# IndigoPurple/DEQSCI

Hardware: AMD Instinct MI355X
Metric: reconstructed frames/sec at 256x256x8, 180 DEQ iters (higher is better)
Workload: dtype f32 (tensors and accumulation; the 64->64 layers' products as split-fp16 MFMAs, see arithmetic)

## Files before the change

deqsci_amd/_hip.py:

```python
import ctypes
import math
import os

import torch

LAYOUT_HWB = 0
LAYOUT_BHW = 1
MAX_M = 8
PART_STRIDE = MAX_M + 1
BN_TRAIN_CHUNK, BN_TRAIN_MAX_WG = 128, 1024
WGRAD_CHAIN = 4096

_LIB_PATH = os.environ.get("DEQSCI_HIP_LIB") or os.path.join(os.path.dirname(os.path.abspath(__file__)), "lib", "libdeqsci_hip.so")
_lib = None

_i64, _int, _f32, _ptr = ctypes.c_int64, ctypes.c_int, ctypes.c_float, ctypes.c_void_p
_f64 = ctypes.c_double

SIGNATURES = {
    "deqsci_sci_forward_f32": [_ptr, _ptr, _ptr, _i64, _i64, _i64, _i64, _int, _int, _ptr],
    "deqsci_sci_adjoint_f32": [_ptr, _ptr, _ptr, _i64, _i64, _i64, _i64, _int, _int, _ptr],
    "deqsci_phi_sum_f32": [_ptr, _ptr, _i64, _i64, _i64, _i64, _int, _ptr],
    "deqsci_gap_update_f32": [_ptr, _ptr, _ptr, _ptr, _ptr, _i64, _i64, _i64, _i64, _int, _int, _int, _ptr],
    "deqsci_gap_update_grad_f32": [_ptr, _ptr, _ptr, _ptr, _ptr, _ptr, _ptr, _ptr, _ptr, _i64, _i64, _i64, _i64, _int, _int, _ptr],
# ... 8 lines not shown
    "deqsci_residual_store_ref_f32": [_ptr, _ptr, _ptr, _ptr, _ptr, _ptr, _ptr, _ptr, _i64, _i64, _int, _int, _int, _ptr],
    "deqsci_anderson_apply_solve_ref_f32": [_ptr, _ptr, _ptr, _ptr, _ptr, _ptr, _i64, _i64, _int, _int, _int, _int, _f32, _f32, _ptr],
    "deqsci_gram_ref_fusable": [_i64, _i64],
    "deqsci_gram_row_chain16_f32": [_ptr, _ptr, _ptr, _i64, _i64, _int, _int, _int, _int, _ptr],
    "deqsci_anderson_mix_f32": [_ptr, _ptr, _ptr, _ptr, _f32, _int, _i64, _i64, _int, _ptr],
    "deqsci_anderson_mix_gap_f32": [_ptr, _ptr, _ptr, _f32, _int, _int, _ptr, _ptr, _ptr, _ptr, _ptr,
                                    _i64, _i64, _i64, _i64, _int, _int, _ptr],
    "deqsci_anderson_mix_gap_timed_f32": [_ptr, _ptr, _ptr, _f32, _int, _int, _ptr, _ptr, _ptr, _ptr, _ptr,
                                          _i64, _i64, _i64, _i64, _int, _int, _ptr, _ptr, _ptr],
    "deqsci_bias_relu_f32": [_ptr, _ptr, _i64, _i64, _i64, _int, _int, _ptr],
    "deqsci_ffdnet_tail_f32": [_ptr, _ptr, _ptr, _ptr, _i64, _i64, _i64, _ptr],
    "deqsci_ffdnet_head_f32": [_ptr, _ptr, _ptr, _i64, _ptr, _i64, _i64, _i64, _ptr],
    "deqsci_conv3x3_c64_to_1_f32": [_ptr, _ptr, _ptr, _ptr, _i64, _i64, _i64, _ptr],
    "deqsci_conv3x3_c1_to_64_f32": [_ptr, _ptr, _ptr, _i64, _i64, _i64, _int, _ptr],
    "deqsci_conv3x3_c64_winograd_f32": [_ptr, _ptr, _ptr, _ptr, _i64, _i64, _i64, _int, _ptr],
    "deqsci_conv3x3_c64_winograd_timed_f32": [_ptr, _ptr, _ptr, _ptr, _i64, _i64, _i64, _int, _ptr, _ptr, _ptr],
    "deqsci_conv3x3_c64_winograd44_f32": [_ptr, _ptr, _ptr, _ptr, _i64, _i64, _i64, _int, _ptr],
    "deqsci_conv3x3_c64_winograd44_timed_f32": [_ptr, _ptr, _ptr, _ptr, _i64, _i64, _i64, _int, _ptr, _ptr, _ptr],
    "deqsci_conv3x3_c64_winograd44_layout_f32": [_ptr, _ptr, _ptr, _ptr, _i64, _i64, _i64, _int, _int, _int, _ptr, _ptr, _ptr],
    "deqsci_conv3x3_c64_split16": [_ptr, _ptr, _ptr, _ptr, _i64, _i64, _i64, _int, _int, _ptr, _int, _ptr, _int, _ptr, _int, _ptr, _ptr, _ptr],
    "deqsci_conv3x3_c64_split16_stack": [_ptr, _ptr, _ptr, _ptr, _int, _i64, _i64, _i64, _ptr, _i64, _int, _int, _ptr, _ptr, _ptr, _ptr],
    "deqsci_conv3x3_c64_wino16": [_ptr, _ptr, _ptr, _ptr, _i64, _i64, _i64, _int, _int, _ptr, _int, _ptr, _int, _ptr, _ptr, _ptr],
    "deqsci_conv3x3_c64_wino16_stack": [_ptr, _ptr, _ptr, _ptr, _int, _i64, _i64, _i64, _ptr, _i64, _int, _int, _ptr, _ptr, _ptr, _ptr],
    "deqsci_f32_to_split16": [_ptr, _ptr, _i64, _i64, _i64, _ptr, _int, _ptr],
    "deqsci_absmax_f32": [_ptr, _i64, _i64, _ptr, _ptr],
    "deqsci_ffdnet_tail_split16": [_ptr, _ptr, _ptr, _i64, _i64, _i64, _int, _ptr, _int, _ptr],
    "deqsci_ffdnet_head_split16": [_ptr, _ptr, _ptr, _i64, _ptr, _i64, _i64, _i64, _int, _ptr, _int, _ptr, _int, _ptr, _ptr],
    "deqsci_conv3x3_c64_to_1_split16": [_ptr, _ptr, _ptr, _i64, _i64, _i64, _int, _ptr, _int, _ptr],
    "deqsci_conv3x3_c64_to_1_p32": [_ptr, _ptr, _ptr, _i64, _i64, _i64, _int, _ptr, _int, _ptr],
    "deqsci_conv3x3_c1_to_64_p32": [_ptr, _ptr, _ptr, _i64, _i64, _i64, _int, _ptr, _int, _ptr, _ptr],
    "deqsci_ffdnet_head_p32": [_ptr, _ptr, _ptr, _i64, _ptr, _i64, _i64, _i64, _int, _ptr, _int, _ptr, _int, _ptr],
    "deqsci_ffdnet_tail_p32": [_ptr, _ptr, _ptr, _i64, _i64, _i64, _int, _ptr, _int, _ptr],
    "deqsci_conv3x3_c1_to_64_sp16": [_ptr, _ptr, _ptr, _i64, _i64, _i64, _int, _ptr, _int, _ptr, _ptr],
    "deqsci_ssim_f32": [_ptr, _ptr, _ptr, _i64, _i64, _i64, _i64, _int, _int, _int, _int, _ptr, _ptr],
    "deqsci_sqerr_rows_f32": [_ptr, _ptr, _ptr, _i64, _i64, _i64, _int, _ptr, _ptr],
    "deqsci_gaptv_f32": [_ptr, _ptr, _ptr, _ptr, _i64, _i64, _i64, _i64, _int, _int, _f64, _f64, _f64, _int, _ptr, _ptr, _ptr],
    "deqsci_tv_chambolle_f32": [_ptr, _ptr, _i64, _i64, _i64, _f64, _f64, _int, _f64, _ptr, _ptr, _ptr],
    "deqsci_relu_mask_pack_f32": [_ptr, _ptr, _i64, _ptr],
    "deqsci_conv3x3_c64_winograd_masked_f32": [_ptr, _ptr, _ptr, _ptr, _i64, _i64, _i64, _ptr],
    "deqsci_conv3x3_c1_to_64_masked_f32": [_ptr, _ptr, _ptr, _ptr, _i64, _i64, _i64, _ptr],
    "deqsci_ffdnet_head_masked_f32": [_ptr, _ptr, _ptr, _ptr, _i64, _i64, _i64, _ptr],
    "deqsci_power_step_f32": [_ptr, _ptr, _ptr, _ptr, _i64, _i64, _ptr, _ptr],
    "deqsci_broyden_dots_f32": [_ptr, _ptr, _ptr, _ptr, _ptr, _ptr, _ptr, _i64, _i64, _int, _int, _ptr],
    "deqsci_broyden_update_f32": [_ptr, _ptr, _ptr, _ptr, _ptr, _ptr, _ptr, _ptr, _ptr, _ptr, _i64, _i64, _int, _int, _int, _ptr],
    "deqsci_epsilon2_norms_f32": [_ptr, _ptr, _ptr, _ptr, _ptr, _i64, _i64, _ptr],
    "deqsci_epsilon2_update_f32": [_ptr, _ptr, _ptr, _ptr, _ptr, _ptr, _i64, _i64, _f32, _ptr],
    "deqsci_wgrad3x3_c64_c64_f32": [_ptr, _ptr, _ptr, _i64, _i64, _i64, _ptr, _ptr],
    "deqsci_wgrad3x3_c1_c64_f32": [_ptr, _ptr, _ptr, _int, _i64, _i64, _i64, _ptr, _ptr],
    "deqsci_wgrad3x3_c64_c64_bn_f32": [_ptr, _ptr, _ptr, _ptr, _ptr, _ptr, _ptr, _i64, _i64, _i64, _ptr, _ptr],
    "deqsci_wgrad3x3_shuffle_f32": [_ptr, _ptr, _i64, _ptr, _ptr, _int, _i64, _i64, _i64, _ptr, _ptr],
    "deqsci_realsn_power_f32": [_ptr, _ptr, _ptr, _ptr, _ptr, _int, _f32, _f32, _i64, _i64, _i64, _i64, _ptr, _ptr],
    "deqsci_realsn_grad_f32": [_ptr, _ptr, _ptr, _ptr, _ptr, _ptr, _f32, _i64, _i64, _i64, _i64, _ptr, _ptr],
    "deqsci_bn_train_stats_f32": [_ptr, _ptr, _ptr, _ptr, _ptr, _f64, _i64, _ptr, _ptr],
    "deqsci_bn_train_apply_f32": [_ptr, _ptr, _ptr, _ptr, _f64, _ptr, _ptr, _int, _i64, _ptr],
    "deqsci_bn_train_grad_stats_f32": [_ptr, _ptr, _ptr, _f64, _ptr, _ptr, _ptr, _i64, _ptr, _ptr],
    "deqsci_bn_train_grad_apply_f32": [_ptr, _ptr, _ptr, _ptr, _ptr, _f64, _ptr, _i64, _ptr],
    "deqsci_event_create": [ctypes.POINTER(_ptr)],
    "deqsci_event_destroy": [_ptr],
    "deqsci_event_elapsed_ms": [_ptr, _ptr, ctypes.POINTER(_f32)],
}
OTHER_EXPORTS = ("deqsci_version", "deqsci_error_string", "deqsci_anderson_chunks",
                 "deqsci_partials_bytes", "deqsci_gram_bytes", "deqsci_gram_ref_bytes", "deqsci_ssim_workspace_bytes",
                 "deqsci_gaptv_workspace_bytes", "deqsci_tv_chambolle_workspace_bytes", "deqsci_sqerr_workspace_bytes", "deqsci_power_workspace_bytes",
                 "deqsci_broyden_workspace_bytes", "deqsci_broyden_chunk", "deqsci_epsilon2_workspace_bytes", "deqsci_epsilon2_chunk",
                 "deqsci_wgrad_workspace_bytes", "deqsci_wgrad_bn_workspace_bytes", "deqsci_realsn_workspace_bytes",
                 "deqsci_bn_train_workspace_bytes")


class DeqsciHipError(RuntimeError):
    pass


def lib_path():
    return _LIB_PATH


def load():
    global _lib
    if _lib is not None:
        return _lib
    if not os.path.exists(_LIB_PATH):
        raise DeqsciHipError(
            f"{_LIB_PATH} is missing: build it with `make` (or __graft_entry__.build()). "
            "deqsci_amd has no CPU / eager fallback for its HIP kernels.")
    lib = ctypes.CDLL(_LIB_PATH, mode=ctypes.RTLD_GLOBAL)
    for name, argtypes in SIGNATURES.items():
        fn = getattr(lib, name)
        fn.argtypes = argtypes
        fn.restype = _int
# ... 14 lines not shown
    lib.deqsci_sqerr_workspace_bytes.argtypes = [_i64, _i64]
    lib.deqsci_power_workspace_bytes.restype = ctypes.c_size_t
    lib.deqsci_power_workspace_bytes.argtypes = [_i64, _i64]
    lib.deqsci_broyden_workspace_bytes.restype = ctypes.c_size_t
    lib.deqsci_broyden_workspace_bytes.argtypes = [_i64, _i64, _int]
    lib.deqsci_broyden_chunk.restype = _i64
    lib.deqsci_broyden_chunk.argtypes = []
    lib.deqsci_epsilon2_workspace_bytes.restype = ctypes.c_size_t
    lib.deqsci_epsilon2_workspace_bytes.argtypes = [_i64, _i64]
    lib.deqsci_epsilon2_chunk.restype = _i64
    lib.deqsci_epsilon2_chunk.argtypes = []
    lib.deqsci_wgrad_workspace_bytes.restype = ctypes.c_size_t
    lib.deqsci_wgrad_workspace_bytes.argtypes = [_i64, _i64, _i64]
    lib.deqsci_wgrad_bn_workspace_bytes.restype = ctypes.c_size_t
    lib.deqsci_wgrad_bn_workspace_bytes.argtypes = [_i64, _i64, _i64]
    lib.deqsci_realsn_workspace_bytes.restype = ctypes.c_size_t
    lib.deqsci_realsn_workspace_bytes.argtypes = [_i64, _i64, _i64, _i64]
    lib.deqsci_bn_train_workspace_bytes.restype = ctypes.c_size_t
    lib.deqsci_bn_train_workspace_bytes.argtypes = [_i64]
    lib.deqsci_gaptv_workspace_bytes.restype = _i64
    lib.deqsci_gaptv_workspace_bytes.argtypes = [_i64, _i64, _i64, _i64]
    lib.deqsci_tv_chambolle_workspace_bytes.restype = _i64
    lib.deqsci_tv_chambolle_workspace_bytes.argtypes = [_i64, _i64, _i64]
    _lib = lib
    return lib


def _check(code, what):
    if code != 0:
        msg = load().deqsci_error_string(code).decode()
        raise DeqsciHipError(f"{what} failed with code {code}: {msg}")


def _p(t, name="tensor", allow_none=False):
    if t is None:
        if allow_none:
            return None
        raise DeqsciHipError(f"{name} is None")
    if not isinstance(t, torch.Tensor) or not t.is_cuda:
        raise DeqsciHipError(f"{name} must be a torch tensor on a HIP device (got "
                             f"{getattr(t, 'device', type(t))}); deqsci_amd has no CPU path")
    if t.dtype != torch.float32:
        raise DeqsciHipError(f"{name} must be float32, got {t.dtype}")
    if not t.is_contiguous():
        raise DeqsciHipError(f"{name} must be contiguous")
    return t.data_ptr()
# ... 925 lines not shown
            raise DeqsciHipError("conv3x3_c64_split16: a measuring launch (track=) serves the sp16 output")
        with _dev(x.t):
            _check(load().deqsci_conv3x3_c64_split16(x.t.data_ptr(), wp.data_ptr(), _p(bias, "bias", True), None, n, H, W, 1 if relu else 0,
                                                     weights.sw, _rng(x.rng, n), x.exp, None, 0, _rng(track, n), 0, _stream(), None, None),
                   "conv3x3_c64_split16 (measuring)")
        return None
    if out_f32:
        o = out if out is not None else torch.empty((n, 64, H, W), dtype=torch.float32, device=dev, memory_format=torch.channels_last)
        ot = o
    else:
        o = out if out is not None else Sp16.empty(n, H, W, dev)
        o.rng, o.exp = out_rng, int(out_exp)
        ot = o.t
    ev = _hook_events("s16", n, H, W, events) or (None, None)
    with _dev(x.t):
        _check(load().deqsci_conv3x3_c64_split16(x.t.data_ptr(), wp.data_ptr(), _p(bias, "bias", True), ot.data_ptr(), n, H, W, 1 if relu else 0,
                                                 weights.sw, _rng(x.rng, n), x.exp, _rng(out_rng, n), int(out_exp), None, 1 if out_f32 else 0,
                                                 _stream(), ev[0], ev[1]), "conv3x3_c64_split16")
    return o


class _Stack:
    __slots__ = ("table", "n_layers", "keep", "_state")

    def __init__(self, layers, device):
        rows, keep = [], []
        for w16, bias, relu in layers:
            if not isinstance(w16, self.WEIGHTS):
                raise DeqsciHipError(f"{type(self).__name__}: every layer needs {self.WEIGHTS.__name__}")
            wp = w16.packed if w16.packed.device == torch.device(device) else w16.packed.to(device)
            b = None if bias is None else f32c(bias.detach().to(device))
            if b is not None and b.numel() < 64:
                raise DeqsciHipError(f"{type(self).__name__}: bias must have 64 elements")
            keep += [wp, b]
            rows += [wp.data_ptr(), 0 if b is None else b.data_ptr(), (int(w16.sw) & 0xffffffff) | ((1 if relu else 0) << 32)]
        self.table = torch.tensor(rows, dtype=torch.int64).to(device)
        self.n_layers, self.keep, self._state = len(layers), keep, {}

    def state(self, n, H, W):
        st = self._state.get(("out", n, H, W))
        if st is None:
            dev = self.table.device
            for key in [k for k in self._state if k[0] == "out"]:
                del self._state[key]
            st = self._state[("out", n, H, W)] = (self.ACT.empty(n, H, W, dev), self.ACT.empty(n, H, W, dev))
        return st

    def head_buffer(self, n, H, W):
        hb = self._state.get(("head", n, H, W))
        if hb is None:
            for key in [k for k in self._state if k[0] == "head"]:
                del self._state[key]
            hb = self._state[("head", n, H, W)] = self.ACT.empty(n, H, W, self.table.device)
        return hb

    def flags(self, n, H, W):
        fl = self._state.get(("flags", n, H, W))
        if fl is None:
            n_tiles = n * (-(-H // self.TILE[0])) * (-(-W // self.TILE[1]))
            fl = self._state[("flags", n, H, W)] = torch.zeros(32 * (n_tiles + 1), dtype=torch.int32, device=self.table.device)
        return fl

    def timed_out(self):
        bad = False
        for key, fl in self._state.items():
            if key[0] == "flags" and int(fl[-32]) != 0:
                fl.zero_()
                bad = True
        return bad


STACK_SLICE_BYTES = 128 << 20


def split16_stack_per_launch(n, H, W, slice_bytes=STACK_SLICE_BYTES, cus=None, tile=(16, 32)):
    per = max(1, int(slice_bytes) // (H * W * 256))
    if cus:
        tiles = (-(-H // tile[0])) * (-(-W // tile[1]))
        unit = int(cus) // math.gcd(tiles, int(cus))
        if per >= unit:
            per -= per % unit
    return min(per, n)


def conv3x3_c64_split16_stack(x, stack, ranges=None, events=None, per_launch=None, rng_offset=0, out_bufs=None, check=None):
    if not isinstance(x, Sp16) or not isinstance(stack, Split16Stack) or not x.t.is_contiguous() or x.t.dtype != torch.float16 or not x.t.is_cuda:
        raise DeqsciHipError("conv3x3_c64_split16_stack: a contiguous Sp16 GPU activation and a Split16Stack are required")
    return _stack_launch("conv3x3_c64_split16_stack", x, stack, ranges, events, per_launch, rng_offset, out_bufs, check)


# ... 549 lines not shown
```

deqsci_amd/csrc/conv_w16.hip:

```cpp
#include "common.hpp"
#include <hip/hip_ext.h>
#include <type_traits>
#pragma clang diagnostic ignored "-Winline-asm"

namespace deqsci {
namespace w16 {

typedef _Float16 h8 __attribute__((ext_vector_type(8)));
typedef float f32x16 __attribute__((ext_vector_type(16)));
typedef float f32x4 __attribute__((ext_vector_type(4)));
typedef float f32x2 __attribute__((ext_vector_type(2)));
typedef int i32x4 __attribute__((ext_vector_type(4)));
typedef unsigned u32x4 __attribute__((ext_vector_type(4)));
typedef __attribute__((address_space(3))) char lds_char;
typedef __attribute__((address_space(3))) u32x4 lds_u32x4;
typedef __attribute__((address_space(3))) f32x4 lds_f32x4;

constexpr int WAVES = 8, TBW = 64 * WAVES;
constexpr int OUT_ROWS = 8, OUT_COLS = 64, RAW_ROWS = 10, RAW_COLS = 66, RAW_HALF = 33, RAW_PIX = RAW_ROWS * RAW_COLS;
constexpr int PLANE_B = RAW_PIX * 16;
constexpr int RAW_SLOTS = 4 * RAW_PIX;
constexpr int RAW_TOTAL = 42;
constexpr int RAW_INSTR = 6;
constexpr int RAW_BUF = RAW_TOTAL * 1024;
constexpr int W_FRAGS = 2 * 3 * 2 * 2;
constexpr int W_HALF = W_FRAGS * 1024;
constexpr int W_INSTR = W_FRAGS / WAVES;
constexpr uint32_t RAW_OOB = 0x80000000u;

__device__ __forceinline__ float sub1(float a, float b) { float r; asm("v_sub_f32 %0, %1, %2" : "=v"(r) : "v"(a), "v"(b)); return r; }
__device__ __forceinline__ float add1(float a, float b) { float r; asm("v_add_f32 %0, %1, %2" : "=v"(r) : "v"(a), "v"(b)); return r; }

__device__ __forceinline__ f32x2 pk_add(f32x2 a, f32x2 b) { f32x2 r; asm("v_pk_add_f32 %0, %1, %2" : "=v"(r) : "v"(a), "v"(b)); return r; }
__device__ __forceinline__ f32x2 pk_sub(f32x2 a, f32x2 b) { f32x2 r; asm("v_pk_add_f32 %0, %1, %2 neg_lo:[0,1] neg_hi:[0,1]" : "=v"(r) : "v"(a), "v"(b)); return r; }
__device__ __forceinline__ f32x2 pk_fma(f32x2 a, f32x2 b, f32x2 c) { f32x2 r; asm("v_pk_fma_f32 %0, %1, %2, %3" : "=v"(r) : "v"(a), "v"(b), "v"(c)); return r; }

struct StackLayer { const char* w; const float* bias; int w_exp; int relu; };
constexpr unsigned STACK_SPIN_LIMIT = 1u << 21;
constexpr int STACK_POLLS = 8;
constexpr int STACK_FLAG_STRIDE = 32;

template <int STACK>
__global__ __launch_bounds__(TBW, 2) void conv_w16_kernel(const char* __restrict__ x, const char* __restrict__ Wp, const float* __restrict__ bias,
                                                          char* __restrict__ y, int H, int W, int relu, int w_exp, const float* __restrict__ in_amax, int in_exp,
                                                          const float* __restrict__ out_amax, int out_exp, int tiles_x, int tiles_y,
                                                          int n_tiles, uint32_t mg_img, uint32_t sh_img, uint32_t mg_tx, uint32_t sh_tx,
                                                          char* __restrict__ y2, const StackLayer* __restrict__ layers, int n_layers, unsigned* flags,
                                                          int range_stride) {
    __shared__ __attribute__((aligned(16))) char Raw[2 * RAW_BUF];
    __shared__ __attribute__((aligned(16))) char Wt[2 * W_HALF];
    __shared__ __attribute__((aligned(16))) float bias_s[STACK ? 128 : 64];
    __shared__ uint32_t ready_s;
    __shared__ uint32_t poll_s[64];
    __shared__ uint32_t voff_s[RAW_INSTR * TBW];
    const int lane = (int)(threadIdx.x & 63);
    const int wave = (int)uniform((uint32_t)(threadIdx.x >> 6));
    int t_first, t_step, t_end;
    {
        const int nb = (int)gridDim.x, b = (int)blockIdx.x;
        if ((nb & 7) == 0) {
            const int per_xcd = (n_tiles + 7) >> 3;
            t_first = (b & 7) * per_xcd + (b >> 3);
            t_step = nb >> 3;
            t_end = min(n_tiles, ((b & 7) + 1) * per_xcd);
        } else { t_first = b; t_step = nb; t_end = n_tiles; }
    }
    if (t_first >= t_end) return;
    const int Wq = tiles_x * OUT_COLS;
    const int64_t HW = (int64_t)H * Wq;
    const int pl = lane & 31, kb = lane >> 5;
    const bool six = wave < RAW_TOTAL - 8 * (RAW_INSTR - 1);
    auto wait_all_but_a_tile = [&]() __attribute__((always_inline)) {
        if (six) asm volatile("s_waitcnt vmcnt(%0)" ::"n"(RAW_INSTR) : "memory");
        else asm volatile("s_waitcnt vmcnt(%0)" ::"n"(RAW_INSTR - 1) : "memory");
    };

    i32x4 rsrc;
    int ft_py0 = 0, ft_px0 = 0;
    auto fetch_tile_uniform = [&](int t, const char* xb) __attribute__((always_inline)) {
        const int n = mdiv(t, mg_img, sh_img), r = t - n * (tiles_x * tiles_y);
        const int by = mdiv(r, mg_tx, sh_tx), bx = r - by * tiles_x;
        const uint64_t base = (uint64_t)(xb + (int64_t)n * HW * 256);
        rsrc.x = (int)uniform((uint32_t)base);
        rsrc.y = (int)uniform((uint32_t)(base >> 32));
        rsrc.z = (int)uniform((uint32_t)(HW * 256));
        rsrc.w = 0x00020000;
        ft_py0 = OUT_ROWS * by - 1;
        ft_px0 = OUT_COLS * bx - 1;
// ... 73 lines not shown
        split_pair(va[2 * s], va[2 * s + 1], hi, lo);
        Vh[ns][0][2 * f + s] = hi; Vl[ns][0][2 * f + s] = lo;
        split_pair(vb[2 * s], vb[2 * s + 1], hi, lo);
        Vh[ns][1][2 * f + s] = hi; Vl[ns][1][2 * f + s] = lo;
    };
    auto xf_step = [&](int i, int rb, int rho, int hh, int ns) __attribute__((always_inline)) {
        if (i == 0) t_load(rb, rho, hh, 0);
        else if (i == 4 || i == 5) t_xf(i - 4, hh);
        else if (i == 6) { t_split(0, ns, 0); t_load(rb, rho, hh, 1); }
        else if (i == 7) t_split(1, ns, 0);
        else if (i == 8 || i == 9) t_xf(i - 8, hh);
        else if (i == 10 || i == 11) t_split(i - 10, ns, 1);
    };
    auto t_row = [&](int rb, int rho, int hh, int ns) __attribute__((always_inline)) {
#pragma unroll
        for (int i = 0; i < 12; ++i) xf_step(i, rb, rho, hh, ns);
    };

#ifdef W16_STAMP
    uint32_t st_sum[8] = {0, 0, 0, 0, 0, 0, 0, 0};
    uint64_t st_t = __builtin_readcyclecounter();
#define W16_MARK(i) do { const uint64_t now_ = __builtin_readcyclecounter(); st_sum[i] += (uint32_t)(now_ - st_t); st_t = now_; } while (0)
    uint32_t* st_out = reinterpret_cast<uint32_t*>(const_cast<float*>(STACK ? layers[0].bias : bias));
#else
#define W16_MARK(i) do { } while (0)
#endif
    int L = 0;
    auto tile_done = [&](int t) -> Done {
        Done d;
        const int n = mdiv(t, mg_img, sh_img), rr_ = t - n * (tiles_x * tiles_y);
        const int by = mdiv(rr_, mg_tx, sh_tx), bx = rr_ - by * tiles_x;
        const int ox = OUT_COLS * bx + 2 * pl;
        const uint64_t ob = (uint64_t)(y + (int64_t)n * HW * 256);
        d.orsrc.x = (int)uniform((uint32_t)ob);
        d.orsrc.y = (int)uniform((uint32_t)(ob >> 32));
        d.orsrc.z = (int)uniform((uint32_t)(HW * 256));
        d.orsrc.w = 0x00020000;
        {
            const int e_in = STACK ? (in_amax ? sp16_act_exp(in_amax[(int64_t)L * range_stride + n]) : L == 0 ? in_exp : out_exp)
                                   : in_amax ? sp16_act_exp(in_amax[n]) : in_exp;
            const int e_out = STACK ? (in_amax ? sp16_act_exp(in_amax[(int64_t)(L + 1) * range_stride + n]) : out_exp)
                                    : out_amax ? sp16_act_exp(out_amax[n]) : out_exp;
            d.oscale = sp16_pow2(e_out - e_in - w_exp);
            d.bscale = sp16_pow2(e_out);
        }
        d.oy = OUT_ROWS * by + wave;
        d.pix[0] = ox >= W ? RAW_OOB : (uint32_t)((kb * (int)HW + OUT_COLS * bx + pl) * 16);
        d.pix[1] = ox + 1 >= W ? RAW_OOB : (uint32_t)((kb * (int)HW + OUT_COLS * bx + 32 + pl) * 16);
        return d;
    };

    const char* Wnx = nullptr;
    bool s3_raw = false;
    const char* s3_w = nullptr;

    u32x4 Alo[2][2], Ahi[2][2];
    auto loadA = [&](int wbuf, int dy, int piece, int xp, int cg) __attribute__((always_inline)) {
        const u32x4 v = *reinterpret_cast<const lds_u32x4*>(abase + wbuf * W_HALF + ((((xp * 3 + dy) * 2 + piece) * 2 + cg) * 1024));
        if (piece) Alo[xp][cg] = v; else Ahi[xp][cg] = v;
    };
    auto half_stage = [&](int hs, bool wnext, bool rnext, bool raw_prev, auto&& before_barrier, auto&& shadow) __attribute__((always_inline)) {
        const int c = hs >> 1, h = hs & 1, wb = hs & 1;
        const int hn = h ^ 1, rbn = (h ? (c + 1) : c) & 1;
        auto dma = [&](int k) __attribute__((always_inline)) {
            if (k < W_INSTR) {
                if (wnext) w_piece((STACK && hs >= 6) ? s3_w : Wp, (hs + 2) & 7, wb, k);
            } else if (h == 1 && k < W_INSTR + RAW_INSTR) { if (rnext) raw_piece((c + 2) & 3, c & 1, k - W_INSTR); }
        };
        const f32x16 zero16 = {0, 0, 0, 0, 0, 0, 0, 0, 0, 0, 0, 0, 0, 0, 0, 0};
#pragma unroll
        for (int dy = 0; dy < 3; ++dy) {
            const int slot = (3 * hs + dy) & 1;
            if (dy == 2) {
                W16_MARK(h);
                if (h == 0 && raw_prev) wait_all_but_a_tile();
                else asm volatile("s_waitcnt vmcnt(0)" ::: "memory");
                W16_MARK(2 + h);
                before_barrier();
                lds_barrier();
                W16_MARK(4);
            }
#pragma unroll
            for (int i = 0; i < 12; ++i) {
                const int m = 12 * dy + i, pass = i >> 2, xp = (i >> 1) & 1, cg = i & 1, xi = 2 * h + xp;
                const bool z1st = c == 0 && dy == 0 && pass == 0;
                const h8 a = __builtin_bit_cast(h8, pass == 0 ? Alo[xp][cg] : Ahi[xp][cg]);
                const h8 b = __builtin_bit_cast(h8, pass == 1 ? Vl[slot][xp] : Vh[slot][xp]);
                acc[xi][cg] = __builtin_amdgcn_mfma_f32_32x32x16_f16(a, b, z1st ? zero16 : acc[xi][cg], 0, 0, 0);
                __builtin_amdgcn_sched_barrier(0);
// ... 53 lines not shown
    first_row_and_fragments();

    auto flag_word = [&](int t) __attribute__((always_inline)) -> const unsigned* {
        const int tpi = tiles_x * tiles_y;
        const int n = mdiv(t, mg_img, sh_img), r = t - n * tpi, by = mdiv(r, mg_tx, sh_tx), bx = r - by * tiles_x;
        const int k = lane < 9 ? lane : 4;
        const int ny = by + k / 3 - 1, nx = bx + k % 3 - 1;
        const bool ok = ny >= 0 && ny < tiles_y && nx >= 0 && nx < tiles_x;
        return flags + (int64_t)(ok ? n * tpi + ny * tiles_x + nx : t) * STACK_FLAG_STRIDE;
    };
    int pend_t = -1;
    unsigned pend_v = 0;
    f32x4 o[2][4][2];
    Done dp = {(i32x4){0, 0, 0, 0}, {RAW_OOB, RAW_OOB}, 0, 0.0f, 0.0f};
    bool have_o = false;
    auto store_step = [&](int k) __attribute__((always_inline)) {
        const int g = k >> 3, gq = (k >> 1) & 3, p = k & 1;
        if (!(dp.oy < H)) return;
        const uint32_t so = uniform((uint32_t)(2 * (4 * g + gq)) * (uint32_t)HW * 16u + (uint32_t)(dp.oy * Wq) * 16u);
        if (STACK) asm volatile("buffer_store_dwordx4 %0, %1, %2, %3 offen sc1\n\ts_nop 1" ::"v"(o[g][gq][p]), "v"(dp.pix[p]), "s"(dp.orsrc), "s"(so) : "memory");
        else asm volatile("buffer_store_dwordx4 %0, %1, %2, %3 offen nt\n\ts_nop 1" ::"v"(o[g][gq][p]), "v"(dp.pix[p]), "s"(dp.orsrc), "s"(so) : "memory");
    };
    bool raw_flying = true;
#pragma unroll 1
    for (int t_cur = t_first;;) {
        const bool new_layer = STACK && !(t_cur + t_step < t_end);
        const int t_next = new_layer ? t_first : t_cur + t_step;
        const bool next = STACK ? (!new_layer || L + 1 < n_layers) : t_next < t_end;
        const int L_next = L + (new_layer ? 1 : 0);
        const bool poll = STACK && next && L_next > 0;
        if (STACK && new_layer && next) Wnx = layers[L + 1].w;
        half_stage(0, true, false, raw_flying, nothing, [&](int m) __attribute__((always_inline)) {
            if ((m & 1) && m < 32 && have_o) store_step(m >> 1);
        });
        have_o = false;
        half_stage(1, true, true, false, nothing, [&](int m) __attribute__((always_inline)) {
            if (STACK && m == 24 && pend_t >= 0 && wave == 2 && lane == 0)
                __hip_atomic_store(flags + (int64_t)pend_t * STACK_FLAG_STRIDE, pend_v, __ATOMIC_RELAXED, __HIP_MEMORY_SCOPE_AGENT);
        });
        pend_t = -1;
        half_stage(2, true, false, true, nothing, no_shadow);
        half_stage(3, true, true, false, nothing, [&](int m) __attribute__((always_inline)) {
            if (STACK && m == 24 && wave == 0 && poll) {
                const unsigned* pf = flag_word(t_next);
                const uint32_t m0v = uniform((uint32_t)(uintptr_t)(__attribute__((address_space(3))) uint32_t*)poll_s);
                asm volatile("s_mov_b32 m0, %0\n\ts_nop 0\n\tglobal_load_lds_dword %1, off sc1" ::"s"(m0v), "v"(pf) : "m0", "memory");
            }
        });
        half_stage(4, true, false, true, [&]() __attribute__((always_inline)) {
            if (STACK && wave == 0) {
                const unsigned pv = poll_s[lane];
                const unsigned target = fbase + (unsigned)L_next;
                const bool late = poll && lane < 9 && (int)(pv - target) < 0;
                const uint32_t ok = (!poll || fgiveup) ? 1u : (__builtin_amdgcn_ballot_w64(late) == 0 ? 1u : 0u);
                if (lane == 0) ready_s = ok;
            }
        }, [&](int m) __attribute__((always_inline)) {
            if (m == 1 && next) fetch_tile_uniform(t_next, (STACK && new_layer) ? y : x);
            if (m >= 2 && m < 2 + 2 * RAW_INSTR && !(m & 1) && next) voff_set((m - 2) >> 1, fetch_lane_offset((m - 2) >> 1));
        });
        bool ready = true;
        if (STACK) {
            ready = uniform(ready_s) != 0;
            s3_raw = next && ready;
            s3_w = new_layer ? Wnx : Wp;
        }
        const bool rn = STACK ? s3_raw : next;
        half_stage(5, true, rn, false, nothing, no_shadow);
        half_stage(6, next, false, rn, nothing, no_shadow);
        half_stage(7, next, rn, false, nothing, [&](int m) __attribute__((always_inline)) { if (m == 28) dp = tile_done(t_cur); });
        raw_flying = rn;

        const bool store_now = STACK ? (!next || !ready) : !next;
        const float floor_ = relu ? 0.0f : -__builtin_inff();
        const __attribute__((address_space(3))) float* bsl = (const __attribute__((address_space(3))) float*)bias_s + (STACK ? 64 * (L & 1) : 0);
#pragma unroll
        for (int g = 0; g < 2; ++g) {
#pragma unroll
            for (int gq = 0; gq < 4; ++gq) {
                const f32x4 bz = *reinterpret_cast<const lds_f32x4*>(bsl + 32 * g + 8 * gq + 4 * kb) * dp.bscale;
#pragma unroll
                for (int k = 0; k < 4; k += 2) {
                    const int i = 4 * gq + k;
                    const f32x2 m0 = {acc[0][g][i], acc[0][g][i + 1]}, m1 = {acc[1][g][i], acc[1][g][i + 1]};
                    const f32x2 m2 = {acc[2][g][i], acc[2][g][i + 1]}, m3 = {acc[3][g][i], acc[3][g][i + 1]};
                    const f32x2 y0 = pk_add(pk_add(m0, m1), m2), y1 = pk_sub(pk_sub(m1, m2), m3);
                    const f32x2 sc = {dp.oscale, dp.oscale}, b2 = {bz[k], bz[k + 1]};
                    const f32x2 z0 = pk_fma(y0, sc, b2), z1 = pk_fma(y1, sc, b2);
                    o[g][gq][0][k] = __builtin_elementwise_maximum(z0.x, floor_);
                    o[g][gq][0][k + 1] = __builtin_elementwise_maximum(z0.y, floor_);
                    o[g][gq][1][k] = __builtin_elementwise_maximum(z1.x, floor_);
                    o[g][gq][1][k + 1] = __builtin_elementwise_maximum(z1.y, floor_);
                }
                if (store_now) { store_step(2 * (4 * g + gq)); store_step(2 * (4 * g + gq) + 1); }
            }
        }
        have_o = !store_now;
        if (rn) wait_all_but_a_tile();
        else asm volatile("s_waitcnt vmcnt(0)" ::: "memory");
        W16_MARK(5);
        if (STACK) {
            const unsigned done_v = fbase + (unsigned)(L + 1);
            if (new_layer && next) {
                const StackLayer ln = layers[L + 1];
                x = y;
                y = ((L + 1) & 1) ? y2 : y_even;
                Wp = ln.w; bias = ln.bias; w_exp = ln.w_exp; relu = ln.relu;
#ifndef W16_STAMP
                if (wave == 1) bias_s[64 * ((L + 1) & 1) + lane] = bias ? bias[lane] : 0.0f;
#endif
            }
            if (next && !ready) {
                if (have_o) {
#pragma unroll
                    for (int k = 0; k < 16; ++k) store_step(k);
                    have_o = false;
                }
                asm volatile("s_waitcnt vmcnt(0)" ::: "memory");
                __syncthreads();
                if (wave == 2 && lane == 0)
                    __hip_atomic_store(flags + (int64_t)t_cur * STACK_FLAG_STRIDE, done_v, __ATOMIC_RELAXED, __HIP_MEMORY_SCOPE_AGENT);
                if (wave == 0) {
                    const unsigned target = fbase + (unsigned)L_next;
                    const unsigned* f = flag_word(t_next);
                    if (!fgiveup) {
                        unsigned v[STACK_POLLS], spins = 0;
#pragma unroll
                        for (int q = 0; q < STACK_POLLS; ++q) {
                            asm volatile("global_load_dword %0, %1, off sc1" : "=v"(v[q]) : "v"(f) : "memory");
                            __builtin_amdgcn_s_sleep(3);
                        }
                        bool waiting = true;
// ... 5 lines not shown
                                if (++spins > STACK_SPIN_LIMIT) {
                                    fgiveup = 1;
                                    if (lane == 0) __hip_atomic_fetch_or(flags + (int64_t)n_tiles * STACK_FLAG_STRIDE, 1u, __ATOMIC_RELAXED, __HIP_MEMORY_SCOPE_AGENT);
                                    waiting = false;
                                    break;
                                }
                                asm volatile("global_load_dword %0, %1, off sc1" : "=v"(v[q]) : "v"(f) : "memory");
                                __builtin_amdgcn_s_sleep(3);
                            }
                        }
                        asm volatile("s_waitcnt vmcnt(0)" ::: "memory");
                    }
                }
                __syncthreads();
                fetch_two_chunks_and_wait();
                __syncthreads();
                first_row_and_fragments();
                raw_flying = true;
                W16_MARK(7);
            } else {
                pend_t = t_cur;
                pend_v = done_v;
            }
            if (new_layer) ++L;
        }
        if (!next) break;
        t_cur = t_next;
    }
    if (have_o) {
#pragma unroll
        for (int k = 0; k < 16; ++k) store_step(k);
    }
    asm volatile("s_waitcnt vmcnt(0)" ::: "memory");
    if (STACK) {
        __syncthreads();
        if (pend_t >= 0 && threadIdx.x == 0)
            __hip_atomic_store(flags + (int64_t)pend_t * STACK_FLAG_STRIDE, pend_v, __ATOMIC_RELAXED, __HIP_MEMORY_SCOPE_AGENT);
    }
#ifdef W16_STAMP
    W16_MARK(6);
    if (lane == 0)
        for (int i = 0; i < 8; ++i) st_out[((int)blockIdx.x * WAVES + wave) * 8 + i] = st_sum[i];
#endif
}

}
}

using namespace deqsci;

static_assert(sizeof(w16::StackLayer) == 24, "the layer table of deqsci_conv3x3_c64_wino16_stack is three 8-byte words per layer");

extern "C" int deqsci_conv3x3_c64_wino16(const void* x_p32, const void* u_packed, const float* bias, void* y_p32, int64_t n, int64_t H, int64_t W,
                                         int relu, int w_exp, const float* in_amax, int in_exp, const float* out_amax, int out_exp,
                                         deqsci_stream_t stream, void* start_event, void* stop_event) {
    if (!x_p32 || !u_packed || !y_p32) return DEQSCI_ERR_NULL;
    if ((start_event == nullptr) != (stop_event == nullptr)) return DEQSCI_ERR_NULL;
    if (n <= 0 || H <= 0 || W <= 0) return DEQSCI_ERR_SHAPE;
    if (x_p32 == y_p32 || sp16_bad_exp(w_exp) || sp16_bad_exp(in_exp) || sp16_bad_exp(out_exp)) return DEQSCI_ERR_UNSUPPORTED;
    if (!aligned16(x_p32) || !aligned16(u_packed) || !aligned16(y_p32)) return DEQSCI_ERR_ALIGN;
    const int64_t tiles_x = ceil_div(W, w16::OUT_COLS), tiles_y = ceil_div(H, w16::OUT_ROWS);
    const int64_t n_tiles = n * tiles_x * tiles_y;
    if (n_tiles > (int64_t)INT32_MAX / 16 || H * tiles_x * w16::OUT_COLS * 256 + 16 > (int64_t)w16::RAW_OOB) return DEQSCI_ERR_UNSUPPORTED;
    hipStream_t st = static_cast<hipStream_t>(stream);
    const int64_t resident = (int64_t)num_cus();
    const dim3 grid((unsigned)(n_tiles < resident ? n_tiles : resident));
    uint32_t mg_img, sh_img, mg_tx, sh_tx;
    mdiv_magic((uint32_t)(tiles_x * tiles_y), &mg_img, &sh_img);
    mdiv_magic((uint32_t)tiles_x, &mg_tx, &sh_tx);
    hipEvent_t ev0 = static_cast<hipEvent_t>(start_event), ev1 = static_cast<hipEvent_t>(stop_event);
    hipExtLaunchKernelGGL((w16::conv_w16_kernel<0>), grid, dim3(w16::TBW), 0, st, ev0, ev1, 0, static_cast<const char*>(x_p32), static_cast<const char*>(u_packed),
                          bias, static_cast<char*>(y_p32), (int)H, (int)W, relu, w_exp, in_amax, in_exp, out_amax, out_exp, (int)tiles_x,
                          (int)tiles_y, (int)n_tiles, mg_img, sh_img, mg_tx, sh_tx, static_cast<char*>(nullptr),
                          static_cast<const w16::StackLayer*>(nullptr), 1, static_cast<unsigned*>(nullptr), 0);
    return launch_status();
}

extern "C" int deqsci_conv3x3_c64_wino16_stack(const void* x_p32, void* y_even, void* y_odd, const void* layers, int n_layers,
                                               int64_t n, int64_t H, int64_t W, const float* ranges, int64_t range_stride, int in_exp, int out_exp,
                                               void* flags, deqsci_stream_t stream, void* start_event, void* stop_event) {
    if (!x_p32 || !y_even || !layers || !flags || (n_layers > 1 && !y_odd)) return DEQSCI_ERR_NULL;
    if ((start_event == nullptr) != (stop_event == nullptr)) return DEQSCI_ERR_NULL;
    if (n <= 0 || H <= 0 || W <= 0 || n_layers <= 0 || (ranges && (range_stride < n || range_stride > INT32_MAX))) return DEQSCI_ERR_SHAPE;
    if (x_p32 == y_even || x_p32 == y_odd || y_even == y_odd || n_layers > 64 || sp16_bad_exp(in_exp) || sp16_bad_exp(out_exp)) return DEQSCI_ERR_UNSUPPORTED;
    if (!aligned16(x_p32) || !aligned16(y_even) || !aligned16(y_odd) || (reinterpret_cast<uintptr_t>(layers) & 7u) || (reinterpret_cast<uintptr_t>(flags) & 3u))
        return DEQSCI_ERR_ALIGN;
    const int64_t tiles_x = ceil_div(W, w16::OUT_COLS), tiles_y = ceil_div(H, w16::OUT_ROWS);
    const int64_t n_tiles = n * tiles_x * tiles_y;
    if (H * tiles_x * w16::OUT_COLS * 256 + 16 > (int64_t)w16::RAW_OOB) return DEQSCI_ERR_UNSUPPORTED;
    if (n_tiles > (int64_t)INT32_MAX / (16 * 32)) return DEQSCI_ERR_UNSUPPORTED;
    static int occ_cache[64] = {0};
    const int64_t fit = resident_workgroups(w16::conv_w16_kernel<1>, w16::TBW, occ_cache);
    if (fit <= 0) return DEQSCI_ERR_UNSUPPORTED;
    const int64_t resident = fit < (int64_t)num_cus() ? fit : (int64_t)num_cus();
    hipStream_t st = static_cast<hipStream_t>(stream);
    uint32_t mg_img, sh_img, mg_tx, sh_tx;
    mdiv_magic((uint32_t)(tiles_x * tiles_y), &mg_img, &sh_img);
    mdiv_magic((uint32_t)tiles_x, &mg_tx, &sh_tx);
    hipEvent_t ev0 = static_cast<hipEvent_t>(start_event), ev1 = static_cast<hipEvent_t>(stop_event);
    hipExtLaunchKernelGGL((w16::conv_w16_kernel<1>), dim3((unsigned)(n_tiles < resident ? n_tiles : resident)), dim3(w16::TBW), 0, st, ev0, ev1, 0,
                          static_cast<const char*>(x_p32), static_cast<const char*>(nullptr), static_cast<const float*>(nullptr), static_cast<char*>(y_even),
                          (int)H, (int)W, 0, 0, ranges, in_exp, static_cast<const float*>(nullptr), out_exp, (int)tiles_x, (int)tiles_y, (int)n_tiles,
                          mg_img, sh_img, mg_tx, sh_tx, static_cast<char*>(y_odd), static_cast<const w16::StackLayer*>(layers), n_layers,
                          static_cast<unsigned*>(flags), (int)range_stride);
    return launch_status();
}
```

include/deqsci_hip.h:

```cpp
#ifndef DEQSCI_HIP_H
#define DEQSCI_HIP_H

#include <stddef.h>
#include <stdint.h>

#ifdef __cplusplus
extern "C" {
#endif

#define DEQSCI_LAYOUT_HWB 0
#define DEQSCI_LAYOUT_BHW 1

#define DEQSCI_MAX_M 8
#define DEQSCI_PART_STRIDE (DEQSCI_MAX_M + 1)

#define DEQSCI_ERR_NULL        (-1)
#define DEQSCI_ERR_SHAPE       (-2)
#define DEQSCI_ERR_ALIGN       (-3)
#define DEQSCI_ERR_UNSUPPORTED (-4)

typedef void* deqsci_stream_t;

const char* deqsci_version(void);
const char* deqsci_error_string(int code);
// ... 101 lines not shown

#define DEQSCI_ACT_NHWC 0
#define DEQSCI_ACT_BLK32 1
int deqsci_conv3x3_c64_winograd44_layout_f32(const float* x, const float* u_packed, const float* bias, float* y,
                                             int64_t n, int64_t H, int64_t W, int relu, int in_layout, int out_layout,
                                             deqsci_stream_t stream, void* start_event, void* stop_event);

#define DEQSCI_SP16_DEFAULT_EXP 8
#define DEQSCI_SP16_TARGET_EXP 11
int deqsci_conv3x3_c64_split16(const void* x_sp16, const void* w_packed, const float* bias, void* y,
                               int64_t n, int64_t H, int64_t W, int relu, int w_exp, const float* in_amax, int in_exp,
                               const float* out_amax, int out_exp, float* track_amax, int out_f32,
                               deqsci_stream_t stream, void* start_event, void* stop_event);
int deqsci_conv3x3_c64_split16_stack(const void* x_sp16, void* y_even, void* y_odd, const void* layers, int n_layers,
                                     int64_t n, int64_t H, int64_t W, const float* ranges, int64_t range_stride, int in_exp, int out_exp,
                                     void* flags, deqsci_stream_t stream, void* start_event, void* stop_event);
int deqsci_conv3x3_c64_wino16(const void* x_p32, const void* u_packed, const float* bias, void* y_p32,
                              int64_t n, int64_t H, int64_t W, int relu, int w_exp, const float* in_amax, int in_exp,
                              const float* out_amax, int out_exp,
                              deqsci_stream_t stream, void* start_event, void* stop_event);
int deqsci_conv3x3_c64_wino16_stack(const void* x_p32, void* y_even, void* y_odd, const void* layers, int n_layers,
                                    int64_t n, int64_t H, int64_t W, const float* ranges, int64_t range_stride, int in_exp, int out_exp,
                                    void* flags, deqsci_stream_t stream, void* start_event, void* stop_event);
int deqsci_f32_to_split16(const float* x_nhwc, void* y_sp16, int64_t n, int64_t H, int64_t W, const float* amax, int exp,
                          deqsci_stream_t stream);
int deqsci_absmax_f32(const float* x, int64_t n, int64_t count, float* amax, deqsci_stream_t stream);
int deqsci_conv3x3_c1_to_64_sp16(const float* x, const float* w_packed, void* h_sp16, int64_t n, int64_t H, int64_t W, int relu,
                                 const float* out_amax, int out_exp, float* track_amax, deqsci_stream_t stream);
int deqsci_conv3x3_c1_to_64_p32(const float* x, const float* w_packed, void* h_p32, int64_t n, int64_t H, int64_t W, int relu,
                                const float* out_amax, int out_exp, float* track_amax, deqsci_stream_t stream);
int deqsci_conv3x3_c64_to_1_p32(const void* x_p32, const void* w_packed, float* out, int64_t n, int64_t H, int64_t W,
                                int w_exp, const float* in_amax, int in_exp, deqsci_stream_t stream);
int deqsci_ffdnet_tail_split16(const void* x_sp16, const void* w_packed, float* out, int64_t n, int64_t H, int64_t W,
                               int w_exp, const float* in_amax, int in_exp, deqsci_stream_t stream);
int deqsci_conv3x3_c64_to_1_split16(const void* x_sp16, const void* w_packed, float* out, int64_t n, int64_t H, int64_t W,
                                    int w_exp, const float* in_amax, int in_exp, deqsci_stream_t stream);
int deqsci_ffdnet_head_split16(const float* x, const void* w_packed, const float* sigma, int64_t sigma_stride, void* h_sp16,
                               int64_t n, int64_t H, int64_t W, int w_exp, const float* in_amax, int in_exp,
                               const float* out_amax, int out_exp, float* track_amax, deqsci_stream_t stream);

int deqsci_ffdnet_head_p32(const float* x, const void* w_packed, const float* sigma, int64_t sigma_stride, void* h_p32,
                           int64_t n, int64_t H, int64_t W, int w_exp, const float* in_amax, int in_exp,
                           const float* out_amax, int out_exp, deqsci_stream_t stream);
int deqsci_ffdnet_tail_p32(const void* x_p32, const void* w_packed, float* out, int64_t n, int64_t H, int64_t W,
                           int w_exp, const float* in_amax, int in_exp, deqsci_stream_t stream);

// ... 99 lines not shown
```

Baseline: 149.9.

## Dynamic ticket-based tile scheduling in persistent wino16 layer-stack kernel

Replaces the static strided tile assignment in the persistent Winograd fp16 conv stack kernel with per-XCD atomic ticket counters, so workgroups claim their next tile dynamically across layers. The intent is to balance load and cut tail idle time when workgroups finish at different rates. Layer transitions now follow from the ticket value, and an extra syncthreads guards reuse of the bias buffer. This adds an atomic per tile and ticket reset logic on the host side, with some risk around ordering against the existing cross-layer readiness flags.

After: 151.1, median of 6. About the same (+0.8%).

```diff
diff --git a/deqsci_amd/_hip.py b/deqsci_amd/_hip.py
--- a/deqsci_amd/_hip.py
+++ b/deqsci_amd/_hip.py
@@ -54,6 +54,8 @@
     "deqsci_conv3x3_c64_split16_stack": [_ptr, _ptr, _ptr, _ptr, _int, _i64, _i64, _i64, _ptr, _i64, _int, _int, _ptr, _ptr, _ptr, _ptr],
     "deqsci_conv3x3_c64_wino16": [_ptr, _ptr, _ptr, _ptr, _i64, _i64, _i64, _int, _int, _ptr, _int, _ptr, _int, _ptr, _ptr, _ptr],
     "deqsci_conv3x3_c64_wino16_stack": [_ptr, _ptr, _ptr, _ptr, _int, _i64, _i64, _i64, _ptr, _i64, _int, _int, _ptr, _ptr, _ptr, _ptr],
+    "deqsci_w16_stack_grid": [_i64, _int],
+    "deqsci_w16_stack_ranges": [_i64, _int, _ptr, _ptr],
     "deqsci_f32_to_split16": [_ptr, _ptr, _i64, _i64, _i64, _ptr, _int, _ptr],
     "deqsci_absmax_f32": [_ptr, _i64, _i64, _ptr, _ptr],
     "deqsci_ffdnet_tail_split16": [_ptr, _ptr, _ptr, _i64, _i64, _i64, _int, _ptr, _int, _ptr],
@@ -96,7 +98,7 @@
                  "deqsci_gaptv_workspace_bytes", "deqsci_tv_chambolle_workspace_bytes", "deqsci_sqerr_workspace_bytes", "deqsci_power_workspace_bytes",
                  "deqsci_broyden_workspace_bytes", "deqsci_broyden_chunk", "deqsci_epsilon2_workspace_bytes", "deqsci_epsilon2_chunk",
                  "deqsci_wgrad_workspace_bytes", "deqsci_wgrad_bn_workspace_bytes", "deqsci_realsn_workspace_bytes",
-                 "deqsci_bn_train_workspace_bytes")
+                 "deqsci_bn_train_workspace_bytes", "deqsci_w16_stack_first_tile")
 
 
 class DeqsciHipError(RuntimeError):
@@ -157,6 +159,8 @@
     lib.deqsci_gaptv_workspace_bytes.argtypes = [_i64, _i64, _i64, _i64]
     lib.deqsci_tv_chambolle_workspace_bytes.restype = _i64
     lib.deqsci_tv_chambolle_workspace_bytes.argtypes = [_i64, _i64, _i64]
+    lib.deqsci_w16_stack_first_tile.restype = _i64
+    lib.deqsci_w16_stack_first_tile.argtypes = [_i64, _int, _int]
     _lib = lib
     return lib
 
@@ -1128,6 +1132,7 @@
 
 class _Stack:
     __slots__ = ("table", "n_layers", "keep", "_state")
+    TICKET_LINES = 8
 
     def __init__(self, layers, device):
         rows, keep = [], []
@@ -1164,14 +1169,21 @@
         fl = self._state.get(("flags", n, H, W))
         if fl is None:
             n_tiles = n * (-(-H // self.TILE[0])) * (-(-W // self.TILE[1]))
-            fl = self._state[("flags", n, H, W)] = torch.zeros(32 * (n_tiles + 1), dtype=torch.int32, device=self.table.device)
+            buf = torch.zeros(32 * (n_tiles + 1 + self.TICKET_LINES), dtype=torch.int32, device=self.table.device)
+            fl = self._state[("flags", n, H, W)] = buf[:32 * (n_tiles + 1)]
+            self._state[("tickets", n, H, W)] = buf[32 * (n_tiles + 1):]
         return fl
+
+    def tickets(self, n, H, W):
+        self.flags(n, H, W)
+        return self._state[("tickets", n, H, W)]
 
     def timed_out(self):
         bad = False
         for key, fl in self._state.items():
             if key[0] == "flags" and int(fl[-32]) != 0:
                 fl.zero_()
+                self._state[("tickets",) + key[1:]].zero_()
                 bad = True
         return bad
 
diff --git a/deqsci_amd/csrc/conv_w16.hip b/deqsci_amd/csrc/conv_w16.hip
--- a/deqsci_amd/csrc/conv_w16.hip
+++ b/deqsci_amd/csrc/conv_w16.hip
@@ -39,6 +39,18 @@
 constexpr unsigned STACK_SPIN_LIMIT = 1u << 21;
 constexpr int STACK_POLLS = 8;
 constexpr int STACK_FLAG_STRIDE = 32;
+constexpr int STACK_TICKET_LINES = 8;
+
+struct StackRange { int first, count; };
+__host__ __device__ inline int stack_range_count(int nb) { return (nb & 7) == 0 ? 8 : 1; }
+__host__ __device__ inline int stack_range_of(int nb, int b) { return (nb & 7) == 0 ? (b & 7) : 0; }
+__host__ __device__ inline int stack_number_in_range(int nb, int b) { return (nb & 7) == 0 ? (b >> 3) : b; }
+__host__ __device__ inline StackRange stack_range(int n_tiles, int nb, int r) {
+    if ((nb & 7) != 0) return StackRange{0, n_tiles};
+    const int per_xcd = (n_tiles + 7) >> 3;
+    const int lo = r * per_xcd < n_tiles ? r * per_xcd : n_tiles, hi = (r + 1) * per_xcd < n_tiles ? (r + 1) * per_xcd : n_tiles;
+    return StackRange{lo, hi - lo};
+}
 
 template <int STACK>
 __global__ __launch_bounds__(TBW, 2) void conv_w16_kernel(const char* __restrict__ x, const char* __restrict__ Wp, const float* __restrict__ bias,
@@ -51,19 +63,23 @@
     __shared__ __attribute__((aligned(16))) char Wt[2 * W_HALF];
     __shared__ __attribute__((aligned(16))) float bias_s[STACK ? 128 : 64];
     __shared__ uint32_t ready_s;
+    __shared__ uint32_t ticket_s;
     __shared__ uint32_t poll_s[64];
     __shared__ uint32_t voff_s[RAW_INSTR * TBW];
     const int lane = (int)(threadIdx.x & 63);
     const int wave = (int)uniform((uint32_t)(threadIdx.x >> 6));
     int t_first, t_step, t_end;
+    int r_cnt, tk_off, tk_line;
     {
         const int nb = (int)gridDim.x, b = (int)blockIdx.x;
-        if ((nb & 7) == 0) {
-            const int per_xcd = (n_tiles + 7) >> 3;
-            t_first = (b & 7) * per_xcd + (b >> 3);
-            t_step = nb >> 3;
-            t_end = min(n_tiles, ((b & 7) + 1) * per_xcd);
-        } else { t_first = b; t_step = nb; t_end = n_tiles; }
+        const int r = stack_range_of(nb, b);
+        const StackRange rg = stack_range(n_tiles, nb, r);
+        t_step = nb / stack_range_count(nb);
+        t_first = rg.first + stack_number_in_range(nb, b);
+        t_end = rg.first + rg.count;
+        r_cnt = rg.count;
+        tk_off = rg.first + min(t_step, rg.count);
+        tk_line = n_tiles + 1 + r;
     }
     if (t_first >= t_end) return;
     const int Wq = tiles_x * OUT_COLS;
@@ -183,6 +199,7 @@
     uint64_t st_t = __builtin_readcyclecounter();
 #define W16_MARK(i) do { const uint64_t now_ = __builtin_readcyclecounter(); st_sum[i] += (uint32_t)(now_ - st_t); st_t = now_; } while (0)
     uint32_t* st_out = reinterpret_cast<uint32_t*>(const_cast<float*>(STACK ? layers[0].bias : bias));
+    const uint64_t st_wall0 = wall_clock64();
 #else
 #define W16_MARK(i) do { } while (0)
 #endif
@@ -211,9 +228,6 @@
         return d;
     };
 
-    const char* Wnx = nullptr;
-    bool s3_raw = false;
-    const char* s3_w = nullptr;
 
     u32x4 Alo[2][2], Ahi[2][2];
     auto loadA = [&](int wbuf, int dy, int piece, int xp, int cg) __attribute__((always_inline)) {
@@ -225,7 +239,7 @@
         const int hn = h ^ 1, rbn = (h ? (c + 1) : c) & 1;
         auto dma = [&](int k) __attribute__((always_inline)) {
             if (k < W_INSTR) {
-                if (wnext) w_piece((STACK && hs >= 6) ? s3_w : Wp, (hs + 2) & 7, wb, k);
+                if (wnext) w_piece(Wp, (hs + 2) & 7, wb, k);
             } else if (h == 1 && k < W_INSTR + RAW_INSTR) { if (rnext) raw_piece((c + 2) & 3, c & 1, k - W_INSTR); }
         };
         const f32x16 zero16 = {0, 0, 0, 0, 0, 0, 0, 0, 0, 0, 0, 0, 0, 0, 0, 0};
@@ -325,23 +339,40 @@
         else asm volatile("buffer_store_dwordx4 %0, %1, %2, %3 offen nt\n\ts_nop 1" ::"v"(o[g][gq][p]), "v"(dp.pix[p]), "s"(dp.orsrc), "s"(so) : "memory");
     };
     bool raw_flying = true;
+    unsigned tk_v = (unsigned)(t_first - tk_off);
+    unsigned tk_keep = r_cnt > t_step ? 0u : (unsigned)r_cnt;
+    asm volatile("" : "+v"(tk_keep));
 #pragma unroll 1
     for (int t_cur = t_first;;) {
-        const bool new_layer = STACK && !(t_cur + t_step < t_end);
-        const int t_next = new_layer ? t_first : t_cur + t_step;
-        const bool next = STACK ? (!new_layer || L + 1 < n_layers) : t_next < t_end;
-        const int L_next = L + (new_layer ? 1 : 0);
-        const bool poll = STACK && next && L_next > 0;
-        if (STACK && new_layer && next) Wnx = layers[L + 1].w;
+        bool new_layer = false, next, poll = false;
+        int t_next, L_next = L;
+        if (!STACK) { t_next = t_cur + t_step; next = t_next < t_end; }
         half_stage(0, true, false, raw_flying, nothing, [&](int m) __attribute__((always_inline)) {
+            if (STACK && m == 24 && wave == 3 && lane == 0) {
+                if (tk_keep == 0) asm volatile("global_atomic_add %0, %1, %2, %3 sc0" : "=v"(tk_v) : "v"(tk_line * (STACK_FLAG_STRIDE * 4)), "v"(1), "s"(flags) : "memory");
+                else tk_v += tk_keep;
+            }
             if ((m & 1) && m < 32 && have_o) store_step(m >> 1);
         });
         have_o = false;
-        half_stage(1, true, true, false, nothing, [&](int m) __attribute__((always_inline)) {
+        half_stage(1, true, true, false, [&]() __attribute__((always_inline)) {
+            if (STACK && wave == 3 && lane == 0) ticket_s = tk_v;
+        }, [&](int m) __attribute__((always_inline)) {
             if (STACK && m == 24 && pend_t >= 0 && wave == 2 && lane == 0)
                 __hip_atomic_store(flags + (int64_t)pend_t * STACK_FLAG_STRIDE, pend_v, __ATOMIC_RELAXED, __HIP_MEMORY_SCOPE_AGENT);
         });
         pend_t = -1;
+        if (STACK) {
+            const int k = (int)uniform(ticket_s);
+            while (L_next < n_layers && k + tk_off >= t_end) { tk_off -= r_cnt; ++L_next; }
+            t_next = k + tk_off;
+            next = L_next < n_layers;
+            new_layer = L_next != L;
+            poll = next && L_next > 0;
+            if (k == n_layers * r_cnt - 1 && threadIdx.x == 0)
+                __hip_atomic_store(flags + (int64_t)tk_line * STACK_FLAG_STRIDE, 0u, __ATOMIC_RELAXED, __HIP_MEMORY_SCOPE_AGENT);
+            if (new_layer && next) x = ((L_next - 1) & 1) ? y2 : y_even;
+        }
         half_stage(2, true, false, true, nothing, no_shadow);
         half_stage(3, true, true, false, nothing, [&](int m) __attribute__((always_inline)) {
             if (STACK && m == 24 && wave == 0 && poll) {
@@ -359,17 +390,14 @@
                 if (lane == 0) ready_s = ok;
             }
         }, [&](int m) __attribute__((always_inline)) {
-            if (m == 1 && next) fetch_tile_uniform(t_next, (STACK && new_layer) ? y : x);
+            if (m == 1 && next) fetch_tile_uniform(t_next, x);
             if (m >= 2 && m < 2 + 2 * RAW_INSTR && !(m & 1) && next) voff_set((m - 2) >> 1, fetch_lane_offset((m - 2) >> 1));
         });
         bool ready = true;
-        if (STACK) {
-            ready = uniform(ready_s) != 0;
-            s3_raw = next && ready;
-            s3_w = new_layer ? Wnx : Wp;
-        }
-        const bool rn = STACK ? s3_raw : next;
+        if (STACK) ready = uniform(ready_s) != 0;
+        const bool rn = next && ready;
         half_stage(5, true, rn, false, nothing, no_shadow);
+        if (STACK && new_layer && next) Wp = layers[L_next].w;
         half_stage(6, next, false, rn, nothing, no_shadow);
         half_stage(7, next, rn, false, nothing, [&](int m) __attribute__((always_inline)) { if (m == 28) dp = tile_done(t_cur); });
         raw_flying = rn;
@@ -405,12 +433,12 @@
         if (STACK) {
             const unsigned done_v = fbase + (unsigned)(L + 1);
             if (new_layer && next) {
-                const StackLayer ln = layers[L + 1];
-                x = y;
-                y = ((L + 1) & 1) ? y2 : y_even;
+                const StackLayer ln = layers[L_next];
+                y = (L_next & 1) ? y2 : y_even;
                 Wp = ln.w; bias = ln.bias; w_exp = ln.w_exp; relu = ln.relu;
+                if (((L_next ^ L) & 1) == 0) __syncthreads();
 #ifndef W16_STAMP
-                if (wave == 1) bias_s[64 * ((L + 1) & 1) + lane] = bias ? bias[lane] : 0.0f;
+                if (wave == 1) bias_s[64 * (L_next & 1) + lane] = bias ? bias[lane] : 0.0f;
 #endif
             }
             if (next && !ready) {
@@ -462,7 +490,7 @@
                 pend_t = t_cur;
                 pend_v = done_v;
             }
-            if (new_layer) ++L;
+            L = L_next;
         }
         if (!next) break;
         t_cur = t_next;
@@ -481,6 +509,10 @@
     W16_MARK(6);
     if (lane == 0)
         for (int i = 0; i < 8; ++i) st_out[((int)blockIdx.x * WAVES + wave) * 8 + i] = st_sum[i];
+    if (STACK && threadIdx.x == 0) {
+        st_out[(int)gridDim.x * WAVES * 8 + 2 * (int)blockIdx.x] = (uint32_t)st_wall0;
+        st_out[(int)gridDim.x * WAVES * 8 + 2 * (int)blockIdx.x + 1] = (uint32_t)wall_clock64();
+    }
 #endif
 }
 
@@ -516,6 +548,30 @@
     return launch_status();
 }
 
+extern "C" int deqsci_w16_stack_grid(int64_t n_tiles, int resident) {
+    if (n_tiles <= 0 || resident <= 0) return 0;
+    return (int)(n_tiles < (int64_t)resident ? n_tiles : (int64_t)resident);
+}
+
+extern "C" int deqsci_w16_stack_ranges(int64_t n_tiles, int grid, int64_t* first, int64_t* count) {
+    if (!first || !count) return DEQSCI_ERR_NULL;
+    if (n_tiles <= 0 || n_tiles > INT32_MAX || grid <= 0) return DEQSCI_ERR_SHAPE;
+    const int nr = w16::stack_range_count(grid);
+    for (int r = 0; r < nr; ++r) {
+        const w16::StackRange rg = w16::stack_range((int)n_tiles, grid, r);
+        first[r] = rg.first;
+        count[r] = rg.count;
+    }
+    return nr;
+}
+
+extern "C" int64_t deqsci_w16_stack_first_tile(int64_t n_tiles, int grid, int block) {
+    if (n_tiles <= 0 || n_tiles > INT32_MAX || grid <= 0 || block < 0 || block >= grid) return -1;
+    const w16::StackRange rg = w16::stack_range((int)n_tiles, grid, w16::stack_range_of(grid, block));
+    const int j = w16::stack_number_in_range(grid, block);
+    return j < rg.count ? (int64_t)rg.first + j : -1;
+}
+
 extern "C" int deqsci_conv3x3_c64_wino16_stack(const void* x_p32, void* y_even, void* y_odd, const void* layers, int n_layers,
                                                int64_t n, int64_t H, int64_t W, const float* ranges, int64_t range_stride, int in_exp, int out_exp,
                                                void* flags, deqsci_stream_t stream, void* start_event, void* stop_event) {
@@ -533,12 +589,13 @@
     const int64_t fit = resident_workgroups(w16::conv_w16_kernel<1>, w16::TBW, occ_cache);
     if (fit <= 0) return DEQSCI_ERR_UNSUPPORTED;
     const int64_t resident = fit < (int64_t)num_cus() ? fit : (int64_t)num_cus();
+    const int grid = deqsci_w16_stack_grid(n_tiles, (int)resident);
     hipStream_t st = static_cast<hipStream_t>(stream);
     uint32_t mg_img, sh_img, mg_tx, sh_tx;
     mdiv_magic((uint32_t)(tiles_x * tiles_y), &mg_img, &sh_img);
     mdiv_magic((uint32_t)tiles_x, &mg_tx, &sh_tx);
     hipEvent_t ev0 = static_cast<hipEvent_t>(start_event), ev1 = static_cast<hipEvent_t>(stop_event);
-    hipExtLaunchKernelGGL((w16::conv_w16_kernel<1>), dim3((unsigned)(n_tiles < resident ? n_tiles : resident)), dim3(w16::TBW), 0, st, ev0, ev1, 0,
+    hipExtLaunchKernelGGL((w16::conv_w16_kernel<1>), dim3((unsigned)grid), dim3(w16::TBW), 0, st, ev0, ev1, 0,
                           static_cast<const char*>(x_p32), static_cast<const char*>(nullptr), static_cast<const float*>(nullptr), static_cast<char*>(y_even),
                           (int)H, (int)W, 0, 0, ranges, in_exp, static_cast<const float*>(nullptr), out_exp, (int)tiles_x, (int)tiles_y, (int)n_tiles,
                           mg_img, sh_img, mg_tx, sh_tx, static_cast<char*>(y_odd), static_cast<const w16::StackLayer*>(layers), n_layers,
diff --git a/include/deqsci_hip.h b/include/deqsci_hip.h
--- a/include/deqsci_hip.h
+++ b/include/deqsci_hip.h
@@ -147,6 +147,9 @@
 int deqsci_conv3x3_c64_wino16_stack(const void* x_p32, void* y_even, void* y_odd, const void* layers, int n_layers,
                                     int64_t n, int64_t H, int64_t W, const float* ranges, int64_t range_stride, int in_exp, int out_exp,
                                     void* flags, deqsci_stream_t stream, void* start_event, void* stop_event);
+int deqsci_w16_stack_grid(int64_t n_tiles, int resident);
+int deqsci_w16_stack_ranges(int64_t n_tiles, int grid, int64_t* first, int64_t* count);
+int64_t deqsci_w16_stack_first_tile(int64_t n_tiles, int grid, int block);
 int deqsci_f32_to_split16(const float* x_nhwc, void* y_sp16, int64_t n, int64_t H, int64_t W, const float* amax, int exp,
                           deqsci_stream_t stream);
 int deqsci_absmax_f32(const float* x, int64_t n, int64_t count, float* amax, deqsci_stream_t stream);
```
